# dream-faster/laplace-gnn-recommendation

Hardware: AMD Instinct MI355X
Metric: positive-edges/sec (train step) (higher is better)
Workload: dtype f32; 1 GPU; LightGCN train step, ONE synthetic bipartite graph 8000000x100000 users x items, 100000000 edges (seed 3, 64 user blocks), sharded by user over 1 GPU(s): 8000000 users / 100000000 edges per GPU, 3-layer D=128, global batch 131072 positive edges, on-device sampling, BPR + dense Adam; BASELINE.json configs[3]; parallelism=1 GPU

## Files before the change

### include/laplace_hip.h

```cpp
#ifndef LAPLACE_HIP_H
#define LAPLACE_HIP_H

#include <stddef.h>
#include <stdint.h>

#ifdef __cplusplus
extern "C" {
#endif

#define MI_ABI_VERSION 9

#define MI_ERR_BAD_ARG      (-1)
#define MI_ERR_TOO_LARGE    (-2)
#define MI_ERR_WORKSPACE    (-3)
#define MI_ERR_UNSUPPORTED  (-4)

typedef void* mi_stream_t;

int         mi_abi_version(void);
const char* mi_error_string(int code);

size_t mi_coo_to_csr_workspace_bytes(int64_t n_rows, int64_t nnz);
int    mi_coo_to_csr_i32(int64_t n_rows, int64_t n_cols, int64_t nnz,
                         const int64_t* row, const int64_t* col,
                         int32_t* rowptr, int32_t* col_out, int32_t* perm,
// ... 36 lines not shown

typedef struct mi_spmm_plan_info {
    int64_t n_long_rows, n_items, n_launch, nnz_long;
    int32_t chunk, band, n_bands, queue_len;
    int32_t queue_start[9];
    int32_t keys_in_second;
} mi_spmm_plan_info;

size_t mi_spmm_plan_workspace_bytes(int64_t n_rows, int64_t nnz);
int    mi_spmm_plan_count(int64_t n_rows, int64_t n_cols, const int32_t* rowptr, const int32_t* col,
                          int32_t chunk, int32_t band, void* ws, size_t ws_bytes,
                          mi_spmm_plan_info* info, mi_stream_t stream);
int    mi_spmm_plan_count_range(int64_t n_rows, int64_t n_cols, const int32_t* rowptr, const int32_t* col,
                                int32_t chunk, int32_t max_deg, int32_t band, void* ws, size_t ws_bytes,
                                mi_spmm_plan_info* info, mi_stream_t stream);
int    mi_spmm_plan_fill(int64_t n_rows, const int32_t* rowptr, const mi_spmm_plan_info* info,
                         mi_spmm_plan* plan, void* ws, size_t ws_bytes, mi_stream_t stream);
size_t mi_spmm_plan_pack_workspace_bytes(int64_t n_launch);
int    mi_spmm_plan_pack_entries(const mi_spmm_plan* plan, int64_t nnz_long, const int32_t* col, const float* val,
                                 int32_t values_only, void* ws, size_t ws_bytes, mi_stream_t stream);
size_t mi_spmm_workspace_bytes(const mi_spmm_plan* plan, int64_t d);

int mi_spmm_csr_f32(int64_t n_rows, int64_t d,
                    const int32_t* rowptr, const int32_t* col, const float* val,
                    const float* X, int64_t ldx,
                    float* Y, int64_t ldy,
                    const float* addend, int64_t lda,
                    float* S, int64_t lds, float scale,
                    const mi_spmm_plan* plan, void* ws, size_t ws_bytes,
                    mi_stream_t stream);
// ... 20 lines not shown
} mi_spmm_sweep;

typedef struct mi_spmm_ex {
    const int32_t* x_map;
    const int32_t* addend_map;
    const int32_t* row_list;
    const int32_t* n_list_dev;
    int64_t        n_list;
    const mi_adam_args* adam;
    int32_t        parts;
    int32_t        hot_rows;
    const mi_spmm_sweep* sweep;
    int32_t        hot_base;
    int32_t        hot_threads;
    const uint32_t* x_bits;
} mi_spmm_ex;
#define MI_SPMM_SHORT_ROWS 1
#define MI_SPMM_SPLIT_ROWS 2

int mi_spmm_csr_ex_f32(int64_t n_rows, int64_t d,
                       const int32_t* rowptr, const int32_t* col, const float* val,
                       const float* X, int64_t ldx,
                       float* Y, int64_t ldy,
                       const float* addend, int64_t lda,
                       float* S, int64_t lds, float scale,
                       const mi_spmm_plan* plan, const mi_spmm_ex* ex,
                       void* ws, size_t ws_bytes, mi_stream_t stream);

int mi_map_live_bits_i32(int64_t n, const int32_t* map, uint32_t* bits, mi_stream_t stream);

// ... 338 lines not shown
```

### laplace-gnn-recommendation_amd/_lib.py

```python
from __future__ import annotations

import ctypes
import os
from ctypes import POINTER, Structure, c_char_p, c_double, c_float, c_int32, c_int64, c_size_t, c_uint32, c_uint64, c_void_p

PKG_DIR = os.path.dirname(os.path.abspath(__file__))
LIB_PATH = os.environ.get("LAPLACE_HIP_LIB") or os.path.join(PKG_DIR, "liblaplace_hip.so")

MI_ABI_VERSION = 9
MI_SPMM_GROUP = 32


class MiError(RuntimeError):
    pass


class SpmmPlanStruct(Structure):
    _fields_ = [
        ("chunk", c_int32), ("n_long_rows", c_int32), ("n_items", c_int32), ("n_launch", c_int32),
        ("long_rows", c_void_p), ("item_ptr", c_void_p), ("items", c_void_p), ("long_index", c_void_p),
        ("band", c_int32), ("n_bands", c_int32),
        ("epos", c_void_p), ("ecol", c_void_p), ("eval", c_void_p),
    ]

# ... 6 lines not shown

class AdamArgs(Structure):
    _fields_ = [("p", c_void_p), ("ldp", c_int64), ("m", c_void_p), ("v", c_void_p), ("reg_w", c_void_p),
                ("lr", c_double), ("beta1", c_double), ("beta2", c_double), ("eps", c_double), ("step", c_int64)]


class SpmmSweepStruct(Structure):
    _fields_ = [("col", c_void_p), ("val", c_void_p), ("stream_ptr", c_void_p), ("slot_of", c_void_p),
                ("n_streams", c_int32), ("n_slots", c_int32), ("progress", c_void_p), ("epoch", c_int32), ("slack", c_int32)]


class SpmmExStruct(Structure):
    _fields_ = [("x_map", c_void_p), ("addend_map", c_void_p), ("row_list", c_void_p), ("n_list_dev", c_void_p),
                ("n_list", c_int64), ("adam", POINTER(AdamArgs)), ("parts", c_int32), ("hot_rows", c_int32),
                ("sweep", POINTER(SpmmSweepStruct)), ("hot_base", c_int32), ("hot_threads", c_int32),
                ("x_bits", c_void_p)]


MI_SPMM_SHORT_ROWS, MI_SPMM_SPLIT_ROWS = 1, 2
MI_ERR_UNSUPPORTED = -4
MI_ERR_WORKSPACE = -3
MI_TOPK_ITEMS_PREPARED = 1


class GemmProblem(Structure):
    _fields_ = [("trans_a", c_int32), ("trans_b", c_int32), ("m", c_int64), ("n", c_int64), ("k", c_int64),
                ("A", c_void_p), ("lda", c_int64), ("B", c_void_p), ("ldb", c_int64),
                ("k2", c_int64), ("A2", c_void_p), ("lda2", c_int64), ("B2", c_void_p), ("ldb2", c_int64),
                ("a_mask", c_void_p), ("bias", c_void_p), ("C", c_void_p), ("ldc", c_int64),
                ("accumulate", c_int32), ("act", c_int32)]

# ... 108 lines not shown

P = c_void_p
_PROTOTYPES = {
    "mi_abi_version": (c_int32, []),
    "mi_error_string": (c_char_p, [c_int32]),
    "mi_coo_to_csr_workspace_bytes": (c_size_t, [c_int64, c_int64]),
    "mi_coo_to_csr_i32": (c_int32, [c_int64, c_int64, c_int64, P, P, P, P, P, P, c_size_t, P]),
    "mi_csr_transpose_workspace_bytes": (c_size_t, [c_int64, c_int64]),
    "mi_csr_transpose_i32": (c_int32, [c_int64, c_int64, c_int64, P, P, P, P, P, P, c_size_t, P]),
    "mi_gather_f32": (c_int32, [c_int64, P, P, P, P]),
    "mi_gcn_norm_csr_f32": (c_int32, [c_int64, c_int64, P, P, P, P, P, P]),
    "mi_scale_csr_f32": (c_int32, [c_int64, c_int64, P, P, P, P, P, P, P]),
    "mi_spmm_plan_workspace_bytes": (c_size_t, [c_int64, c_int64]),
    "mi_spmm_plan_count": (c_int32, [c_int64, c_int64, P, P, c_int32, c_int32, P, c_size_t, POINTER(SpmmPlanInfo), P]),
    "mi_spmm_plan_count_range": (c_int32, [c_int64, c_int64, P, P, c_int32, c_int32, c_int32, P, c_size_t, POINTER(SpmmPlanInfo), P]),
    "mi_spmm_plan_fill": (c_int32, [c_int64, P, POINTER(SpmmPlanInfo), POINTER(SpmmPlanStruct), P, c_size_t, P]),
    "mi_spmm_workspace_bytes": (c_size_t, [POINTER(SpmmPlanStruct), c_int64]),
    "mi_spmm_plan_pack_workspace_bytes": (c_size_t, [c_int64]),
    "mi_spmm_plan_pack_entries": (c_int32, [POINTER(SpmmPlanStruct), c_int64, c_void_p, c_void_p, c_int32, c_void_p, c_size_t, c_void_p]),
    "mi_map_live_bits_i32": (c_int32, [c_int64, c_void_p, c_void_p, c_void_p]),
    "mi_spmm_csr_f32": (c_int32, [c_int64, c_int64, P, P, P, P, c_int64, P, c_int64, P, c_int64, P, c_int64,
                                  c_float, POINTER(SpmmPlanStruct), P, c_size_t, P]),
    "mi_spmm_csr_ex_f32": (c_int32, [c_int64, c_int64, P, P, P, P, c_int64, P, c_int64, P, c_int64, P, c_int64,
                                     c_float, POINTER(SpmmPlanStruct), POINTER(SpmmExStruct), P, c_size_t, P]),
    "mi_gather_rows_f32": (c_int32, [c_int64, P, P, c_int64, P, c_int64, P, c_int64, P, c_int64, c_int32, c_float, P]),
    "mi_scatter_rows_f32": (c_int32, [c_int64, P, P, c_int64, P, c_int64, P, c_int64, P, c_int64, P]),
    "mi_batch_nodes_workspace_bytes": (c_size_t, [c_int64]),
    "mi_batch_nodes_i32": (c_int32, [c_int64, c_int64, c_int64, P, P, P, P, P, P, P, c_size_t, P]),
    "mi_csr_expand_rows": (c_int32, [c_int64, P, P, c_int64, P]),
    "mi_sample_bpr_batch": (c_int32, [c_int64, c_int64, P, P, P, c_int64, c_int32, c_int32, c_uint64, c_uint64,
# ... 113 lines not shown
```

### laplace-gnn-recommendation_amd/csrc/spmm.hip

```cpp
#include "common.hpp"
#include "pairs.hpp"
#include <algorithm>
#include <rocprim/rocprim.hpp>

namespace {

#ifndef MI_SPMM_UNROLL
#define MI_SPMM_UNROLL 4
#endif
#ifndef MI_SPMM_UNROLL_ADAM
#define MI_SPMM_UNROLL_ADAM 8
#endif
#ifndef MI_SPMM_UNROLL_PAIR
#define MI_SPMM_UNROLL_PAIR 8
#endif
#ifndef MI_SPMM_ROWS_RPS
#define MI_SPMM_ROWS_RPS 1
#endif
#ifndef MI_SPMM_NT
#define MI_SPMM_NT 0
#endif
typedef float mi_f4v __attribute__((ext_vector_type(4)));
#ifndef MI_SPMM_SC1
#define MI_SPMM_SC1 6
// ... 36 lines not shown
    float4* v;
    const float* reg_w;
    MiAdamConsts adam;
};

struct Ex {
    const int32_t* x_map;
    const int32_t* addend_map;
    const int32_t* row_list;
    const int32_t* n_list_dev;
    const int32_t* long_index;
    int32_t parts;
    int32_t hot_base, hot_rows, hot_threads;
    const uint32_t* x_bits;
    uint8_t* slot_live;
};

template <int LPR>
__device__ __forceinline__ int wave_max_over_subgroups(int n) {
#pragma unroll
    for (int m = MI_WAVE / 2; m >= LPR; m >>= 1) n = max(n, __shfl_xor(n, m, MI_WAVE));
    return n;
}

template <int LPR, int VPL, int UNROLL, bool SPARSE>
__device__ __forceinline__ void subgroup_accumulate(const int32_t* __restrict__ col,
                                                    const float* __restrict__ val,
                                                    const float4* __restrict__ X4, int64_t ldx4, int d4,
                                                    int32_t beg, int n, int nmax, int li,
                                                    const int32_t* __restrict__ x_map, float4 (&acc)[VPL]) {
// ... 187 lines not shown
    const float4* X4; int64_t ldx4;
    Epilogue ep;
};
template <int LPR, int UNROLL>
__global__ __launch_bounds__(kBlock) void spmm_rows_pair_kernel(RowsSide a, RowsSide b, unsigned split) {
    const bool first = blockIdx.x < split;
#define MI_PICK(f) (first ? a.f : b.f)
    Epilogue ep;
    ep.Y = MI_PICK(ep.Y);           ep.ldy4 = MI_PICK(ep.ldy4);
    ep.addend = MI_PICK(ep.addend); ep.lda4 = MI_PICK(ep.lda4);
    ep.S = MI_PICK(ep.S);           ep.lds4 = MI_PICK(ep.lds4);
    ep.scale = MI_PICK(ep.scale);
    ep.streaming = MI_PICK(ep.streaming);
    ep.p = nullptr; ep.ldp4 = 0; ep.m = nullptr; ep.v = nullptr; ep.reg_w = nullptr;
    ep.adam = MiAdamConsts{};
    const Ex ex = {nullptr, nullptr, nullptr, nullptr, nullptr, 0, 0, 0, 0, nullptr, nullptr};
    spmm_rows_body<LPR, 1, UNROLL, MI_SPMM_ROWS_RPS, false, false>(first ? blockIdx.x : blockIdx.x - split, first ? split : gridDim.x - split,
                                                                  MI_PICK(n_out), MI_PICK(d4), MI_PICK(rowptr), MI_PICK(col), MI_PICK(val),
                                                                  MI_PICK(X4), MI_PICK(ldx4), ep, INT32_MAX, ex, 1);
#undef MI_PICK
}


struct HotRows {
    int32_t base, n;
    int32_t row_bytes;
};

#define MI_HOT_ENTRY(U)                                                                                              \
    "v_subrev_u32_e32 %[t2], %[hbase], %[c" #U "]\n"       \
    "v_cmp_gt_u32_e32 vcc, %[hn], %[t2]\n"                 \
// ... 572 lines not shown
    }
    __syncthreads();
    if (wave != 0 || lane >= LPR) return;
    float4 a[VPL];
    load_addend<LPR, VPL>(ep, ar, d4, lane, a);
#pragma unroll
    for (int v = 0; v < VPL; ++v) {
        float4 t = red[0][v][lane];
#pragma unroll
        for (int w = 1; w < kWavesPerBlock; ++w) t = mi_f4_add(t, red[w][v][lane]);
        acc[v] = t;
    }
    store_epilogue<LPR, VPL, ADAM>(ep, out_row, d4, lane, acc, a);
}

struct PlanWs {
    int32_t *is_long, *ldeg, *long_off, *lnz_off;
    int32_t* qstart;
    char* tmp; size_t tmp_bytes;
    int32_t *lrows, *lprefix;
    int32_t *flags, *seg_of;
    int32_t* seg_start;
    uint64_t *keys0, *keys1;
};

size_t plan_tmp_bytes(int64_t n_max) { return mi_align_up((size_t)n_max * 2 + ((size_t)32 << 20), 256); }

bool plan_carve(MiArena& ar, int64_t n_rows, int64_t nnz_total, int64_t n_long, int64_t nnz_long, int64_t n_seg,
                PlanWs& w) {
    const size_t n1 = (size_t)n_rows + 1;
// ... 6 lines not shown
    w.tmp = ar.take<char>(w.tmp_bytes);
    if (!w.is_long || !w.ldeg || !w.long_off || !w.lnz_off || !w.qstart || !w.tmp) return false;
    if (n_long < 0) return true;
    w.lrows = ar.take<int32_t>((size_t)n_long + 1);
    w.lprefix = ar.take<int32_t>((size_t)n_long + 1);
    w.flags = ar.take<int32_t>((size_t)(nnz_long > 0 ? nnz_long : 1));
    w.seg_of = ar.take<int32_t>((size_t)(nnz_long > 0 ? nnz_long : 1));
    if (!w.lrows || !w.lprefix || !w.flags || !w.seg_of) return false;
    if (n_seg < 0) return true;
    w.seg_start = ar.take<int32_t>((size_t)(n_seg > 0 ? n_seg : 1));
    w.keys0 = ar.take<uint64_t>((size_t)(n_seg > 0 ? n_seg : 1));
    w.keys1 = ar.take<uint64_t>((size_t)(n_seg > 0 ? n_seg : 1));
    return w.seg_start && w.keys0 && w.keys1;
}

__global__ void plan_flags_kernel(int64_t n_rows, const int32_t* __restrict__ rowptr, int32_t chunk, int32_t max_deg,
                                  int32_t* __restrict__ is_long, int32_t* __restrict__ ldeg) {
    int64_t r = (int64_t)blockIdx.x * blockDim.x + threadIdx.x;
    if (r > n_rows) return;
    const int32_t deg = (r < n_rows) ? rowptr[r + 1] - rowptr[r] : 0;
    const bool lg = deg > chunk && deg <= max_deg;
    is_long[r] = lg ? 1 : 0;
    ldeg[r] = lg ? deg : 0;
}

__global__ void plan_long_rows_kernel(int64_t n_rows, const int32_t* __restrict__ is_long,
                                      const int32_t* __restrict__ long_off, const int32_t* __restrict__ lnz_off,
                                      int32_t* __restrict__ lrows, int32_t* __restrict__ lprefix) {
    int64_t r = (int64_t)blockIdx.x * blockDim.x + threadIdx.x;
    if (r > n_rows) return;
    if (r == n_rows) {
        lprefix[long_off[r]] = lnz_off[r];
        return;
    }
    if (is_long[r]) {
        lrows[long_off[r]] = (int32_t)r;
// ... 144 lines not shown
}

dim3 plan_grid(int64_t n) { return dim3((unsigned)mi_ceil_div(n > 0 ? n : 1, 256)); }

#ifndef MI_SPMM_HOT_WAVES
#define MI_SPMM_HOT_WAVES 20
#endif
struct HotLaunch { int state = 0; int cus = 0; size_t lds_cap = 0; int occ_key = -1; int occ = 0; };

template <int LPR, int VPL, bool SPARSE, bool ADAM>
int launch_spmm_mode(int64_t n_rows, int d4, const int32_t* rowptr, const int32_t* col, const float* val,
                     const float4* X4, int64_t ldx4, const Epilogue& ep, const mi_spmm_plan* plan,
                     float4* partial, const Ex& ex, int64_t n_list, hipStream_t s, const mi_spmm_sweep* sweep) {
    constexpr int UNROLL = (VPL == 1) ? MI_SPMM_UNROLL : 4;
    constexpr int UNROLL_ROWS = (VPL == 1) ? (ADAM ? MI_SPMM_UNROLL_ADAM : MI_SPMM_UNROLL) : 4;
    constexpr int SG = (MI_WAVE / LPR) * kWavesPerBlock;
    constexpr int ROWS_RPS = MI_SPMM_ROWS_RPS;
#ifndef MI_SPMM_ITEMS_SLOTS
#define MI_SPMM_ITEMS_SLOTS 8
#endif
    constexpr int ITEMS_RPS = (SG >= MI_SPMM_ITEMS_SLOTS) ? 1 : MI_SPMM_ITEMS_SLOTS / SG;
    const int32_t chunk = plan ? plan->chunk : INT32_MAX;
    const bool listed = SPARSE && ex.row_list != nullptr;
    const bool do_short = (ex.parts & MI_SPMM_SHORT_ROWS) != 0, do_split = (ex.parts & MI_SPMM_SPLIT_ROWS) != 0;
    if (do_split && plan && plan->n_items > 0 && sweep) {
        if constexpr (VPL == 1 && LPR <= 32) {
            constexpr int NB = MI_WAVE / LPR;
            const int threads = 32 / NB * MI_WAVE;
            const size_t lds = (size_t)32 * 8 * LPR * sizeof(float4);
            auto kern = spmm_sweep_kernel<LPR, UNROLL, SPARSE>;
// ... 19 lines not shown
        bool done = false;
        xmap_form = false;
        if constexpr (SPARSE) {
            if (ex.x_map && ex.x_bits && ex.slot_live && plan->epos) {
                hipLaunchKernelGGL((spmm_items_xscan_kernel<LPR, VPL>),
                                   dim3((unsigned)mi_ceil_div(n_launch, (int64_t)(kWavesPerBlock * MI_WAVE))), dim3(kBlock), 0, s,
                                   n_launch, d4, reinterpret_cast<const int4*>(plan->items), plan->epos, plan->ecol, plan->eval,
                                   X4, ldx4, partial, ex.x_map, ex.x_bits, ex.slot_live, ep.streaming);
                done = xmap_form = true;
            }
        }
        if (!done)
            hipLaunchKernelGGL((spmm_items_kernel<LPR, VPL, UNROLL, ITEMS_RPS, SPARSE>), gi, dim3(kBlock), 0, s, n_launch,
                               plan->band > 0 ? 1 : 0, d4, reinterpret_cast<const int4*>(plan->items), plan->epos, ecol, eval,
                               X4, ldx4, partial, ex.x_map, ep.streaming);
    }
    const int64_t n_out = listed ? n_list : n_rows;
    bool short_done = false;
    if constexpr (!SPARSE && VPL == 1) {
        if (do_short && n_out > 0 && plan && ex.hot_rows != 0) {
            auto kern = spmm_rows_hot_kernel<LPR, UNROLL, ADAM>;
            static HotLaunch hl;
            const int thr_arg = ex.hot_threads & 0xFFF, waves_arg = ex.hot_threads >> 12;
            const int threads = thr_arg == 512 ? 512 : (thr_arg == 1024 ? 1024 : 256);
            const size_t row_bytes = (size_t)d4 * sizeof(float4);
            if (hl.state == 0) {
                hl.state = -1;
                hipDeviceProp_t prop;
                int dev = 0;
                if (hipGetDevice(&dev) == hipSuccess && hipGetDeviceProperties(&prop, dev) == hipSuccess) {
// ... 71 lines not shown
    if (n_rows < 0 || nnz < 0) return 0;
    const size_t n1 = (size_t)n_rows + 1, z = (size_t)(nnz > 0 ? nnz : 1);
    return 4 * mi_align_up(n1 * 4, 256) + 256 + plan_tmp_bytes(nnz > n_rows + 1 ? nnz : n_rows + 1) +
           2 * mi_align_up(n1 * 4, 256) + 3 * mi_align_up(z * 4, 256) + 2 * mi_align_up(z * 8, 256);
}

int mi_spmm_plan_count(int64_t n_rows, int64_t n_cols, const int32_t* rowptr, const int32_t* col,
                       int32_t chunk, int32_t band, void* ws, size_t ws_bytes, mi_spmm_plan_info* info,
                       mi_stream_t stream) {
    return mi_spmm_plan_count_range(n_rows, n_cols, rowptr, col, chunk, INT32_MAX, band, ws, ws_bytes, info, stream);
}

int mi_spmm_plan_count_range(int64_t n_rows, int64_t n_cols, const int32_t* rowptr, const int32_t* col,
                             int32_t chunk, int32_t max_deg, int32_t band, void* ws, size_t ws_bytes,
                             mi_spmm_plan_info* info, mi_stream_t stream) {
    MI_CHECK_ARG(n_rows >= 0 && n_cols >= 0 && rowptr && chunk > 0 && max_deg >= chunk && band >= 0 && ws && info);
    if (n_rows >= INT32_MAX || n_cols >= INT32_MAX) return MI_ERR_TOO_LARGE;
    hipStream_t s = (hipStream_t)stream;
    memset(info, 0, sizeof(*info));
    info->chunk = chunk;
    info->band = band;
    info->n_bands = band > 0 ? (int32_t)mi_ceil_div(n_cols > 0 ? n_cols : 1, band) : 0;
    int32_t nnz32 = 0;
    MI_HIP(hipMemcpyAsync(&nnz32, rowptr + n_rows, sizeof(int32_t), hipMemcpyDeviceToHost, s));
    MI_HIP(hipStreamSynchronize(s));
    const int64_t nnz = nnz32;
    MI_CHECK_ARG(band == 0 || col || nnz == 0);
    PlanWs w{};
    {
        MiArena ar(ws, ws_bytes);
        if (!plan_carve(ar, n_rows, nnz, -1, -1, -1, w)) return MI_ERR_WORKSPACE;
    }
    const int64_t n1 = n_rows + 1;
    hipLaunchKernelGGL(plan_flags_kernel, plan_grid(n1), dim3(256), 0, s, n_rows, rowptr, chunk, max_deg, w.is_long, w.ldeg);
    size_t tb = w.tmp_bytes;
    MI_HIP(rocprim::exclusive_scan(w.tmp, tb, w.is_long, w.long_off, 0, (size_t)n1, rocprim::plus<int32_t>(), s));
    tb = w.tmp_bytes;
    MI_HIP(rocprim::exclusive_scan(w.tmp, tb, w.ldeg, w.lnz_off, 0, (size_t)n1, rocprim::plus<int32_t>(), s));
    int32_t totals[2] = {0, 0};
    MI_HIP(hipMemcpyAsync(&totals[0], w.long_off + n_rows, sizeof(int32_t), hipMemcpyDeviceToHost, s));
    MI_HIP(hipMemcpyAsync(&totals[1], w.lnz_off + n_rows, sizeof(int32_t), hipMemcpyDeviceToHost, s));
    MI_HIP(hipStreamSynchronize(s));
    const int32_t n_long = totals[0], nnz_long = totals[1];
    info->n_long_rows = n_long;
    info->nnz_long = nnz_long;
    if (n_long == 0) return mi_launch_status();
    {
        MiArena ar(ws, ws_bytes);
        if (!plan_carve(ar, n_rows, nnz, n_long, nnz_long, -1, w)) return MI_ERR_WORKSPACE;
// ... 119 lines not shown
int mi_spmm_csr_ex_f32(int64_t n_rows, int64_t d, const int32_t* rowptr, const int32_t* col,
                       const float* val, const float* X, int64_t ldx, float* Y, int64_t ldy,
                       const float* addend, int64_t lda, float* S, int64_t lds, float scale,
                       const mi_spmm_plan* plan, const mi_spmm_ex* exh, void* ws, size_t ws_bytes,
                       mi_stream_t stream) {
    MI_CHECK_ARG(n_rows >= 0 && d > 0 && rowptr);
    if (n_rows == 0) return 0;
    if (d % 4 != 0 || d > 512) return MI_ERR_UNSUPPORTED;
    if (n_rows >= INT32_MAX) return MI_ERR_TOO_LARGE;
    const mi_adam_args* adam = exh ? exh->adam : nullptr;
    MI_CHECK_ARG(X && (Y || S || adam));
    MI_CHECK_ARG(ldx % 4 == 0 && ldx >= d && mi_aligned16(X));
    MI_CHECK_ARG(!Y || (ldy % 4 == 0 && ldy >= d && mi_aligned16(Y) && Y != X));
    MI_CHECK_ARG(!S || (lds % 4 == 0 && lds >= d && mi_aligned16(S) && S != X));
    MI_CHECK_ARG(!addend || (lda % 4 == 0 && lda >= d && mi_aligned16(addend)));
    Ex ex = {nullptr, nullptr, nullptr, nullptr, nullptr, MI_SPMM_SHORT_ROWS | MI_SPMM_SPLIT_ROWS, 0, 0, 0, nullptr, nullptr};
    int64_t n_list = 0;
    if (exh) {
        ex.x_map = exh->x_map;
        ex.addend_map = exh->addend_map;
        ex.row_list = exh->row_list;
        ex.n_list_dev = exh->n_list_dev;
        n_list = exh->n_list;
        if (exh->parts) {
            MI_CHECK_ARG((exh->parts & ~(MI_SPMM_SHORT_ROWS | MI_SPMM_SPLIT_ROWS)) == 0);
            ex.parts = exh->parts;
        }
        if (!ex.x_map && !ex.row_list && d <= 256) {
            MI_CHECK_ARG(exh->hot_base >= 0 && exh->hot_threads >= 0);
            ex.hot_base = exh->hot_base;
            ex.hot_rows = exh->hot_rows;
            ex.hot_threads = exh->hot_threads;
        }
        if (ex.row_list) {
            MI_CHECK_ARG(n_list >= 0 && !ex.addend_map);
            if (n_list == 0) return 0;
            if (plan && plan->n_long_rows > 0) {
                MI_CHECK_ARG(plan->long_index);
                ex.long_index = plan->long_index;
            }
        }
    }
    const mi_spmm_sweep* sweep = (exh && plan && plan->n_items > 0) ? exh->sweep : nullptr;
    if (sweep) {
        MI_CHECK_ARG(sweep->col && sweep->val && sweep->stream_ptr && sweep->slot_of);
        MI_CHECK_ARG(sweep->n_streams > 0 && sweep->n_streams % 32 == 0 && sweep->n_streams <= 32 * 32);
        MI_CHECK_ARG(sweep->n_slots > 0 && n_cols_ok(sweep) &&
                     (plan->items ? plan->n_items > 8 * sweep->n_slots : plan->n_items == 8 * sweep->n_slots));
        MI_CHECK_ARG(sweep->slack >= 0);
        if (d > 128) return MI_ERR_UNSUPPORTED;
    }
    float4* partial = nullptr;
// ... 100 lines not shown
```

### laplace-gnn-recommendation_amd/ops.py

```python
from __future__ import annotations

import ctypes
import os
from os import environ as _os_environ
from dataclasses import dataclass, field
from typing import Optional, Tuple

import torch as t
from torch import Tensor

from . import _lib
from ._lib import SpmmExStruct, SpmmPlanStruct, SpmmSweepStruct, check

DEFAULT_CHUNK = 256
DEFAULT_BAND = int(_os_environ.get("LAPLACE_SPMM_BAND", 16384))
MIN_BANDED_COLS = 131072

SPMM_EVENTS = None

SPMM_TWO_STREAMS = int(os.environ.get("LAPLACE_SPMM_TWO_STREAMS", "1") or 0)
PACK_ENTRIES = os.environ.get("LAPLACE_SPMM_PACK", "1") != "0"
X_RARE_BITS = os.environ.get("LAPLACE_X_RARE", "1") != "0"
_SIDE = {}


def _side_stream(device) -> "t.cuda.Stream":
    key = t.device(device).index
    if key not in _SIDE:
        _SIDE[key] = t.cuda.Stream(device=device)
    return _SIDE[key]

# ... 58 lines not shown

@dataclass
class SpmmPlan:
    struct: SpmmPlanStruct
    long_rows: Optional[Tensor]
    item_ptr: Optional[Tensor]
    items: Optional[Tensor]
    long_index: Optional[Tensor] = None
    partial: dict = field(default_factory=dict)
    sweep: Optional[SpmmSweepStruct] = None
    sweep_t: tuple = ()
    wide: Optional["SpmmPlan"] = None
    packed: tuple = ()
    packed_of: tuple = ()
    nnz_long: int = 0

    @property
    def n_long_rows(self) -> int:
        return int(self.struct.n_long_rows)

    @property
    def n_items(self) -> int:
        return int(self.struct.n_items)


@dataclass
class DeviceCSR:
    n_rows: int
    n_cols: int
    rowptr: Tensor
    col: Tensor
    val: Optional[Tensor] = None
    perm: Optional[Tensor] = None
    plan: Optional[SpmmPlan] = None
# ... 262 lines not shown
    st.n_items, st.n_launch = off + int(info.n_items), nlaunch
    st.long_rows, st.item_ptr, st.items, st.long_index = long_rows.data_ptr(), item_ptr.data_ptr(), items.data_ptr(), long_index.data_ptr()
    st.band, st.n_bands = int(info.band), int(info.n_bands)
    return SpmmPlan(st, long_rows, item_ptr, items, long_index, sweep=sw.sweep, sweep_t=sw.sweep_t)


HYBRID_TAIL_BAND = int(_os_environ.get("LAPLACE_HYBRID_TAIL_BAND", 16384))


import os as _os
SWEEP = _os.environ.get("LAPLACE_SWEEP", "1") != "0"
SWEEP_BAND = int(_os.environ.get("LAPLACE_SWEEP_BAND", SWEEP_BAND))
SWEEP_PACE = int(_os.environ.get("LAPLACE_SWEEP_PACE", SWEEP_PACE))


def build_spmm_plan(a: DeviceCSR, chunk: int = DEFAULT_CHUNK, band: Optional[int] = None, sweep: Optional[bool] = None) -> SpmmPlan:
    if (SWEEP if sweep is None else sweep) and band is None:
        plan = build_sweep_plan(a, chunk, band=SWEEP_BAND)
        if plan is not None:
            return plan
    L = _lib.lib()
    if band is None:
        band = DEFAULT_BAND if a.n_cols >= MIN_BANDED_COLS else 0
    dev = a.device
    ws = _ws(L.mi_spmm_plan_workspace_bytes(a.n_rows, a.nnz), dev)
    info = _lib.SpmmPlanInfo()
    check(L.mi_spmm_plan_count(a.n_rows, a.n_cols, _ptr(a.rowptr), _ptr(a.col), chunk, band, ws.data_ptr(), ws.numel(),
                               ctypes.byref(info), _stream()), "mi_spmm_plan_count")
    nl, nlaunch = int(info.n_long_rows), int(info.n_launch)
    long_rows = t.empty(max(nl, 1), dtype=t.int32, device=dev)
    item_ptr = t.empty(max(nl, 1) + 1, dtype=t.int32, device=dev)
    items = t.empty(4 * max(nlaunch, 1), dtype=t.int32, device=dev)
    long_index = t.empty(max(a.n_rows, 1), dtype=t.int32, device=dev)
    st = SpmmPlanStruct()
    st.long_rows, st.item_ptr, st.items = long_rows.data_ptr(), item_ptr.data_ptr(), items.data_ptr()
    st.long_index = long_index.data_ptr()
    check(L.mi_spmm_plan_fill(a.n_rows, _ptr(a.rowptr), ctypes.byref(info), ctypes.byref(st), ws.data_ptr(), ws.numel(),
                              _stream()), "mi_spmm_plan_fill")
    plan = SpmmPlan(st, long_rows, item_ptr, items, long_index)
    plan.nnz_long = int(info.nnz_long)
    del ws
    if PACK_ENTRIES and nlaunch > 0 and plan.nnz_long > 0 and a.val is not None:
        _pack_plan_entries(a, plan, values_only=False)
    return plan


def _pack_plan_entries(a: DeviceCSR, plan: SpmmPlan, values_only: bool) -> None:
    L = _lib.lib()
    dev, st = a.device, plan.struct
    if not values_only:
        plan.packed = (t.empty(int(st.n_launch), dtype=t.int32, device=dev), t.empty(plan.nnz_long, dtype=t.int32, device=dev),
                       t.empty(plan.nnz_long, dtype=t.float32, device=dev))
        st.epos, st.ecol, st.eval = (x.data_ptr() for x in plan.packed)
    ws = _ws(L.mi_spmm_plan_pack_workspace_bytes(int(st.n_launch)), dev)
    check(L.mi_spmm_plan_pack_entries(ctypes.byref(st), plan.nnz_long, _ptr(a.col), _ptr(a.val), 1 if values_only else 0,
                                      ws.data_ptr(), ws.numel(), _stream()), "mi_spmm_plan_pack_entries")
# ... 41 lines not shown
            raise ValueError(f"adam.p/m/v must be [{a.n_rows}, {d}]")
        rw = adam.get("reg_w")
        if rw is not None:
            _need(rw, t.float32, "adam.reg_w")
        adam_args = _lib.AdamArgs(p_.data_ptr(), ldp, m_.data_ptr(), v_.data_ptr(), _ptr(rw), float(adam["lr"]),
                                  float(adam.get("beta1", 0.9)), float(adam.get("beta2", 0.999)),
                                  float(adam.get("eps", 1e-8)), int(adam["step"]))
    ldy = _rows_ok(Y, "Y") if Y is not None else 0
    lda = _rows_ok(addend, "addend") if addend is not None else 0
    lds = _rows_ok(S, "S") if S is not None else 0
    if a.plan is None and (a.nnz >= PLAN_MIN_NNZ or row_list is not None):
        a.plan = build_spmm_plan(a)
    plan = a.plan
    if plan is not None and plan.sweep is not None and d > 128:
        if plan.wide is None:
            plan.wide = build_spmm_plan(a, chunk=int(plan.struct.chunk), sweep=False)
        plan = plan.wide
    L = _lib.lib()
    if plan is not None and plan.packed and plan.packed_of != (a.val.data_ptr(), a.val._version):
        _pack_plan_entries(a, plan, values_only=True)
    ws_ptr, ws_bytes = None, 0
    if plan is not None and plan.n_items > 0:
        if d not in plan.partial:
            plan.partial[d] = _ws(L.mi_spmm_workspace_bytes(ctypes.byref(plan.struct), d), a.device)
        ws_ptr, ws_bytes = plan.partial[d].data_ptr(), plan.partial[d].numel()
    col_ptr = _ptr(a.col) if a.nnz else a.rowptr.data_ptr()
    val_ptr = _ptr(a.val) if a.nnz else a.rowptr.data_ptr()
    ev = None
    if SPMM_EVENTS is not None:
        ev = (t.cuda.Event(enable_timing=True), t.cuda.Event(enable_timing=True))
        ev[0].record()
# ... 3 lines not shown
            and PERSISTENT_ROWS):
        hot_base, hot_rows = int(a.hot[0]), int(a.hot[1])
        if hot_rows == 0:
            hot_rows = -1
        if hot_base < 0 or hot_rows < -1 or hot_base + max(hot_rows, 0) > X.shape[0]:
            raise ValueError(f"hot rows [{hot_base}, {hot_base + hot_rows}) lie outside X ({X.shape[0]} rows)")

    x_bits = None
    if (x_rare and X_RARE_BITS and x_map is not None and row_list is None and sweep is None and plan is not None
            and plan.n_items > 0):
        x_bits = getattr(a, "_x_bits", None)
        if x_bits is None:
            x_bits = a._x_bits = t.empty((a.n_cols + 31) // 32, dtype=t.int32, device=a.device)
        check(L.mi_map_live_bits_i32(a.n_cols, _ptr(x_map), _ptr(x_bits), _stream()), "mi_map_live_bits_i32")

    def launch(parts: int, stream: int) -> None:
        exs = None
        if (x_map is not None or addend_map is not None or row_list is not None or adam_args is not None or parts
                or sweep is not None or hot_rows != 0 or HOT_THREADS):
            exs = SpmmExStruct(_ptr(x_map), _ptr(addend_map), _ptr(row_list), _ptr(n_list_dev),
                               row_list.numel() if row_list is not None else 0,
                               ctypes.pointer(adam_args) if adam_args is not None else None, parts, hot_rows,
                               ctypes.pointer(sweep) if sweep is not None else None, hot_base, HOT_THREADS, _ptr(x_bits))
        check(L.mi_spmm_csr_ex_f32(a.n_rows, d, _ptr(a.rowptr), col_ptr, val_ptr, X.data_ptr(), ldx,
                                   _ptr(Y), ldy, _ptr(addend), lda, _ptr(S), lds, float(scale),
                                   ctypes.byref(plan.struct) if plan is not None else None,
                                   ctypes.byref(exs) if exs is not None else None, ws_ptr, ws_bytes,
                                   stream), "mi_spmm_csr_ex_f32")

    if SPMM_TWO_STREAMS and plan is not None and plan.n_items > 0:
        cur = t.cuda.current_stream()
        side = _side_stream(a.device)
        side.wait_stream(cur)
        if SPMM_TWO_STREAMS == 2:
            launch(_lib.MI_SPMM_SPLIT_ROWS, cur.cuda_stream)
            launch(_lib.MI_SPMM_SHORT_ROWS, side.cuda_stream)
        else:
            launch(_lib.MI_SPMM_SHORT_ROWS, side.cuda_stream)
            launch(_lib.MI_SPMM_SPLIT_ROWS, cur.cuda_stream)
        cur.wait_stream(side)
    else:
        launch(0, _stream())
    if ev is not None:
        ev[1].record()
        kind = "sparse" if (x_map is not None or row_list is not None) else ("dense_adam" if adam is not None else "dense")
# ... 475 lines not shown
```

Measured before the change: 2.530 million positive-edges/s.

## Route medium-degree rows to a thin SpMM kernel splitting each row across waves

Adds a thin-row class to the SpMM plan: rows with degree between the chunk size and a threshold tied to the band count are taken out of the banded items path. They are handled by a new kernel that splits each row's nonzeros across one to four waves and reduces the partial sums in shared memory before the epilogue. The aim is to avoid the partial-buffer and item-scheduling overhead of the banded split path for moderately long rows. In exchange it adds a new launch, host-side nonzero and argsort work at plan build, and the ABI version is bumped.

```diff
diff --git a/include/laplace_hip.h b/include/laplace_hip.h
--- a/include/laplace_hip.h
+++ b/include/laplace_hip.h
@@ -8,7 +8,7 @@
 extern "C" {
 #endif
 
-#define MI_ABI_VERSION 9
+#define MI_ABI_VERSION 10
 
 #define MI_ERR_BAD_ARG      (-1)
 #define MI_ERR_TOO_LARGE    (-2)
@@ -75,6 +75,9 @@
 int    mi_spmm_plan_count_range(int64_t n_rows, int64_t n_cols, const int32_t* rowptr, const int32_t* col,
                                 int32_t chunk, int32_t max_deg, int32_t band, void* ws, size_t ws_bytes,
                                 mi_spmm_plan_info* info, mi_stream_t stream);
+int    mi_spmm_plan_count_thin(int64_t n_rows, int64_t n_cols, const int32_t* rowptr, const int32_t* col,
+                               int32_t chunk, int32_t thin_max, int32_t max_deg, int32_t band, void* ws, size_t ws_bytes,
+                               mi_spmm_plan_info* info, mi_stream_t stream);
 int    mi_spmm_plan_fill(int64_t n_rows, const int32_t* rowptr, const mi_spmm_plan_info* info,
                          mi_spmm_plan* plan, void* ws, size_t ws_bytes, mi_stream_t stream);
 size_t mi_spmm_plan_pack_workspace_bytes(int64_t n_launch);
@@ -125,6 +128,8 @@
     int32_t        hot_base;
     int32_t        hot_threads;
     const uint32_t* x_bits;
+    const int32_t* thin_rows;
+    int32_t        n_thin;
 } mi_spmm_ex;
 #define MI_SPMM_SHORT_ROWS 1
 #define MI_SPMM_SPLIT_ROWS 2
diff --git a/laplace-gnn-recommendation_amd/_lib.py b/laplace-gnn-recommendation_amd/_lib.py
--- a/laplace-gnn-recommendation_amd/_lib.py
+++ b/laplace-gnn-recommendation_amd/_lib.py
@@ -7,7 +7,7 @@
 PKG_DIR = os.path.dirname(os.path.abspath(__file__))
 LIB_PATH = os.environ.get("LAPLACE_HIP_LIB") or os.path.join(PKG_DIR, "liblaplace_hip.so")
 
-MI_ABI_VERSION = 9
+MI_ABI_VERSION = 10
 MI_SPMM_GROUP = 32
 
 
@@ -44,7 +44,7 @@
     _fields_ = [("x_map", c_void_p), ("addend_map", c_void_p), ("row_list", c_void_p), ("n_list_dev", c_void_p),
                 ("n_list", c_int64), ("adam", POINTER(AdamArgs)), ("parts", c_int32), ("hot_rows", c_int32),
                 ("sweep", POINTER(SpmmSweepStruct)), ("hot_base", c_int32), ("hot_threads", c_int32),
-                ("x_bits", c_void_p)]
+                ("x_bits", c_void_p), ("thin_rows", c_void_p), ("n_thin", c_int32)]
 
 
 MI_SPMM_SHORT_ROWS, MI_SPMM_SPLIT_ROWS = 1, 2
@@ -183,6 +183,7 @@
     "mi_spmm_plan_workspace_bytes": (c_size_t, [c_int64, c_int64]),
     "mi_spmm_plan_count": (c_int32, [c_int64, c_int64, P, P, c_int32, c_int32, P, c_size_t, POINTER(SpmmPlanInfo), P]),
     "mi_spmm_plan_count_range": (c_int32, [c_int64, c_int64, P, P, c_int32, c_int32, c_int32, P, c_size_t, POINTER(SpmmPlanInfo), P]),
+    "mi_spmm_plan_count_thin": (c_int32, [c_int64, c_int64, P, P, c_int32, c_int32, c_int32, c_int32, P, c_size_t, POINTER(SpmmPlanInfo), P]),
     "mi_spmm_plan_fill": (c_int32, [c_int64, P, POINTER(SpmmPlanInfo), POINTER(SpmmPlanStruct), P, c_size_t, P]),
     "mi_spmm_workspace_bytes": (c_size_t, [POINTER(SpmmPlanStruct), c_int64]),
     "mi_spmm_plan_pack_workspace_bytes": (c_size_t, [c_int64]),
diff --git a/laplace-gnn-recommendation_amd/csrc/spmm.hip b/laplace-gnn-recommendation_amd/csrc/spmm.hip
--- a/laplace-gnn-recommendation_amd/csrc/spmm.hip
+++ b/laplace-gnn-recommendation_amd/csrc/spmm.hip
@@ -74,6 +74,8 @@
     int32_t hot_base, hot_rows, hot_threads;
     const uint32_t* x_bits;
     uint8_t* slot_live;
+    const int32_t* thin_rows;
+    int32_t n_thin;
 };
 
 template <int LPR>
@@ -291,7 +293,7 @@
     ep.streaming = MI_PICK(ep.streaming);
     ep.p = nullptr; ep.ldp4 = 0; ep.m = nullptr; ep.v = nullptr; ep.reg_w = nullptr;
     ep.adam = MiAdamConsts{};
-    const Ex ex = {nullptr, nullptr, nullptr, nullptr, nullptr, 0, 0, 0, 0, nullptr, nullptr};
+    const Ex ex = {nullptr, nullptr, nullptr, nullptr, nullptr, 0, 0, 0, 0, nullptr, nullptr, nullptr, 0};
     spmm_rows_body<LPR, 1, UNROLL, MI_SPMM_ROWS_RPS, false, false>(first ? blockIdx.x : blockIdx.x - split, first ? split : gridDim.x - split,
                                                                   MI_PICK(n_out), MI_PICK(d4), MI_PICK(rowptr), MI_PICK(col), MI_PICK(val),
                                                                   MI_PICK(X4), MI_PICK(ldx4), ep, INT32_MAX, ex, 1);
@@ -894,6 +896,80 @@
     store_epilogue<LPR, VPL, ADAM>(ep, out_row, d4, lane, acc, a);
 }
 
+#ifndef MI_SPMM_UNROLL_THIN
+#define MI_SPMM_UNROLL_THIN 4
+#endif
+#ifndef MI_SPMM_THIN_WAVES
+#define MI_SPMM_THIN_WAVES 1
+#endif
+template <int LPR, int VPL, int UNROLL, bool SPARSE, bool ADAM>
+__global__ __launch_bounds__(kBlock) void spmm_thin_kernel(int64_t n_slots, int32_t waves, int d4,
+                                                           const int32_t* __restrict__ rowptr,
+                                                           const int32_t* __restrict__ col,
+                                                           const float* __restrict__ val,
+                                                           const float4* __restrict__ X4, int64_t ldx4,
+                                                           Epilogue ep, Ex ex) {
+    constexpr int NB = MI_WAVE / LPR, SG = NB * kWavesPerBlock;
+    __shared__ float4 red[SG][VPL][LPR];
+    const int lane = mi_lane();
+    const int li = lane % LPR;
+    const int wave = threadIdx.x / MI_WAVE;
+    const int sgi = wave * NB + lane / LPR;
+    const int pieces = waves * NB;
+    const int first_sg = (wave / waves) * pieces;
+    const int piece = sgi - first_sg;
+    const int64_t q = (int64_t)blockIdx.x * (kWavesPerBlock / waves) + wave / waves;
+    const bool listed = SPARSE && ex.row_list != nullptr;
+    int64_t r = 0, out_row = 0, ar = -1;
+    bool mine = q < n_slots;
+    if (mine) {
+        if (listed) {
+            if (ex.n_list_dev && q >= (int64_t)*ex.n_list_dev) mine = false;
+            if (mine) {
+                r = ex.row_list[q];
+                mine = ex.long_index[r] == -2;
+                out_row = ar = q;
+            }
+        } else {
+            r = ex.thin_rows[q];
+            out_row = r;
+            ar = ex.addend_map ? (int64_t)ex.addend_map[r] : r;
+        }
+    }
+    int32_t beg = 0;
+    int n = 0;
+    if (mine) {
+        const int32_t rb = rowptr[r];
+        const int32_t len = rowptr[r + 1] - rb;
+        const int32_t per = (len + pieces - 1) / pieces;
+        const int32_t b = min(piece * per, len);
+        beg = rb + b;
+        n = min(per, len - b);
+    }
+    const int nmax = wave_max_over_subgroups<LPR>(n);
+    float4 acc[VPL];
+    subgroup_accumulate<LPR, VPL, UNROLL, SPARSE>(col, val, X4, ldx4, d4, beg, n, nmax, li, ex.x_map, acc);
+#pragma unroll
+    for (int v = 0; v < VPL; ++v) red[sgi][v][li] = acc[v];
+    __syncthreads();
+    if (!mine || piece != 0) return;
+    float4 a[VPL];
+    load_addend<LPR, VPL>(ep, ar, d4, li, a);
+#pragma unroll
+    for (int v = 0; v < VPL; ++v) {
+        float4 t = red[first_sg][v][li];
+        for (int g = 1; g < pieces; ++g) t = mi_f4_add(t, red[first_sg + g][v][li]);
+        acc[v] = t;
+    }
+    store_epilogue<LPR, VPL, ADAM>(ep, out_row, d4, li, acc, a);
+}
+
+int32_t thin_waves() {
+    const char* e = getenv("LAPLACE_SPMM_THIN_WAVES");
+    const int v = e ? atoi(e) : MI_SPMM_THIN_WAVES;
+    return (v == 1 || v == 2) ? v : 4;
+}
+
 struct PlanWs {
     int32_t *is_long, *ldeg, *long_off, *lnz_off;
     int32_t* qstart;
@@ -930,12 +1006,12 @@
     return w.seg_start && w.keys0 && w.keys1;
 }
 
-__global__ void plan_flags_kernel(int64_t n_rows, const int32_t* __restrict__ rowptr, int32_t chunk, int32_t max_deg,
+__global__ void plan_flags_kernel(int64_t n_rows, const int32_t* __restrict__ rowptr, int32_t min_deg, int32_t max_deg,
                                   int32_t* __restrict__ is_long, int32_t* __restrict__ ldeg) {
     int64_t r = (int64_t)blockIdx.x * blockDim.x + threadIdx.x;
     if (r > n_rows) return;
     const int32_t deg = (r < n_rows) ? rowptr[r + 1] - rowptr[r] : 0;
-    const bool lg = deg > chunk && deg <= max_deg;
+    const bool lg = deg > min_deg && deg <= max_deg;
     is_long[r] = lg ? 1 : 0;
     ldeg[r] = lg ? deg : 0;
 }
@@ -1110,6 +1186,7 @@
                      float4* partial, const Ex& ex, int64_t n_list, hipStream_t s, const mi_spmm_sweep* sweep) {
     constexpr int UNROLL = (VPL == 1) ? MI_SPMM_UNROLL : 4;
     constexpr int UNROLL_ROWS = (VPL == 1) ? (ADAM ? MI_SPMM_UNROLL_ADAM : MI_SPMM_UNROLL) : 4;
+    constexpr int UNROLL_THIN = (VPL == 1) ? MI_SPMM_UNROLL_THIN : 4;
     constexpr int SG = (MI_WAVE / LPR) * kWavesPerBlock;
     constexpr int ROWS_RPS = MI_SPMM_ROWS_RPS;
 #ifndef MI_SPMM_ITEMS_SLOTS
@@ -1159,6 +1236,14 @@
             hipLaunchKernelGGL((spmm_items_kernel<LPR, VPL, UNROLL, ITEMS_RPS, SPARSE>), gi, dim3(kBlock), 0, s, n_launch,
                                plan->band > 0 ? 1 : 0, d4, reinterpret_cast<const int4*>(plan->items), plan->epos, ecol, eval,
                                X4, ldx4, partial, ex.x_map, ep.streaming);
+    }
+    if (do_split && ex.n_thin > 0) {
+        const int32_t waves = thin_waves();
+        const int64_t n_slots = listed ? n_list : (int64_t)ex.n_thin;
+        if (n_slots > 0)
+            hipLaunchKernelGGL((spmm_thin_kernel<LPR, VPL, UNROLL_THIN, SPARSE, ADAM>),
+                               dim3((unsigned)mi_ceil_div(n_slots, (int64_t)(kWavesPerBlock / waves))), dim3(kBlock), 0, s, n_slots,
+                               waves, d4, rowptr, col, val, X4, ldx4, ep, ex);
     }
     const int64_t n_out = listed ? n_list : n_rows;
     bool short_done = false;
@@ -1260,7 +1345,15 @@
 int mi_spmm_plan_count_range(int64_t n_rows, int64_t n_cols, const int32_t* rowptr, const int32_t* col,
                              int32_t chunk, int32_t max_deg, int32_t band, void* ws, size_t ws_bytes,
                              mi_spmm_plan_info* info, mi_stream_t stream) {
+    return mi_spmm_plan_count_thin(n_rows, n_cols, rowptr, col, chunk, 0, max_deg, band, ws, ws_bytes, info, stream);
+}
+
+int mi_spmm_plan_count_thin(int64_t n_rows, int64_t n_cols, const int32_t* rowptr, const int32_t* col,
+                            int32_t chunk, int32_t thin_max, int32_t max_deg, int32_t band, void* ws, size_t ws_bytes,
+                            mi_spmm_plan_info* info, mi_stream_t stream) {
     MI_CHECK_ARG(n_rows >= 0 && n_cols >= 0 && rowptr && chunk > 0 && max_deg >= chunk && band >= 0 && ws && info);
+    MI_CHECK_ARG(thin_max == 0 || (thin_max >= chunk && thin_max <= max_deg));
+    const int32_t min_deg = std::max(chunk, thin_max);
     if (n_rows >= INT32_MAX || n_cols >= INT32_MAX) return MI_ERR_TOO_LARGE;
     hipStream_t s = (hipStream_t)stream;
     memset(info, 0, sizeof(*info));
@@ -1278,7 +1371,7 @@
         if (!plan_carve(ar, n_rows, nnz, -1, -1, -1, w)) return MI_ERR_WORKSPACE;
     }
     const int64_t n1 = n_rows + 1;
-    hipLaunchKernelGGL(plan_flags_kernel, plan_grid(n1), dim3(256), 0, s, n_rows, rowptr, chunk, max_deg, w.is_long, w.ldeg);
+    hipLaunchKernelGGL(plan_flags_kernel, plan_grid(n1), dim3(256), 0, s, n_rows, rowptr, min_deg, max_deg, w.is_long, w.ldeg);
     size_t tb = w.tmp_bytes;
     MI_HIP(rocprim::exclusive_scan(w.tmp, tb, w.is_long, w.long_off, 0, (size_t)n1, rocprim::plus<int32_t>(), s));
     tb = w.tmp_bytes;
@@ -1428,7 +1521,7 @@
     MI_CHECK_ARG(!Y || (ldy % 4 == 0 && ldy >= d && mi_aligned16(Y) && Y != X));
     MI_CHECK_ARG(!S || (lds % 4 == 0 && lds >= d && mi_aligned16(S) && S != X));
     MI_CHECK_ARG(!addend || (lda % 4 == 0 && lda >= d && mi_aligned16(addend)));
-    Ex ex = {nullptr, nullptr, nullptr, nullptr, nullptr, MI_SPMM_SHORT_ROWS | MI_SPMM_SPLIT_ROWS, 0, 0, 0, nullptr, nullptr};
+    Ex ex = {nullptr, nullptr, nullptr, nullptr, nullptr, MI_SPMM_SHORT_ROWS | MI_SPMM_SPLIT_ROWS, 0, 0, 0, nullptr, nullptr, nullptr, 0};
     int64_t n_list = 0;
     if (exh) {
         ex.x_map = exh->x_map;
@@ -1446,10 +1539,15 @@
             ex.hot_rows = exh->hot_rows;
             ex.hot_threads = exh->hot_threads;
         }
+        if (exh->n_thin > 0) {
+            MI_CHECK_ARG(plan && exh->thin_rows);
+            ex.thin_rows = exh->thin_rows;
+            ex.n_thin = exh->n_thin;
+        }
         if (ex.row_list) {
             MI_CHECK_ARG(n_list >= 0 && !ex.addend_map);
             if (n_list == 0) return 0;
-            if (plan && plan->n_long_rows > 0) {
+            if (plan && (plan->n_long_rows > 0 || ex.n_thin > 0)) {
                 MI_CHECK_ARG(plan->long_index);
                 ex.long_index = plan->long_index;
             }
diff --git a/laplace-gnn-recommendation_amd/ops.py b/laplace-gnn-recommendation_amd/ops.py
--- a/laplace-gnn-recommendation_amd/ops.py
+++ b/laplace-gnn-recommendation_amd/ops.py
@@ -15,6 +15,7 @@
 DEFAULT_CHUNK = 256
 DEFAULT_BAND = int(_os_environ.get("LAPLACE_SPMM_BAND", 16384))
 MIN_BANDED_COLS = 131072
+THIN_PER_BAND = int(_os_environ.get("LAPLACE_SPMM_THIN", 2))
 
 SPMM_EVENTS = None
 
@@ -103,10 +104,20 @@
     packed: tuple = ()
     packed_of: tuple = ()
     nnz_long: int = 0
+    thin_rows: Optional[Tensor] = None
+    thin_max: int = 0
+
+    @property
+    def n_thin_rows(self) -> int:
+        return int(self.thin_rows.numel()) if self.thin_rows is not None else 0
+
+    @property
+    def n_split_rows(self) -> int:
+        return int(self.struct.n_long_rows)
 
     @property
     def n_long_rows(self) -> int:
-        return int(self.struct.n_long_rows)
+        return int(self.struct.n_long_rows) + self.n_thin_rows
 
     @property
     def n_items(self) -> int:
@@ -399,7 +410,8 @@
 SWEEP_PACE = int(_os.environ.get("LAPLACE_SWEEP_PACE", SWEEP_PACE))
 
 
-def build_spmm_plan(a: DeviceCSR, chunk: int = DEFAULT_CHUNK, band: Optional[int] = None, sweep: Optional[bool] = None) -> SpmmPlan:
+def build_spmm_plan(a: DeviceCSR, chunk: int = DEFAULT_CHUNK, band: Optional[int] = None, sweep: Optional[bool] = None,
+                    thin_max: Optional[int] = None) -> SpmmPlan:
     if (SWEEP if sweep is None else sweep) and band is None:
         plan = build_sweep_plan(a, chunk, band=SWEEP_BAND)
         if plan is not None:
@@ -407,11 +419,16 @@
     L = _lib.lib()
     if band is None:
         band = DEFAULT_BAND if a.n_cols >= MIN_BANDED_COLS else 0
+        if thin_max is None and band > 0:
+            thin_max = THIN_PER_BAND * ((a.n_cols + band - 1) // band)
+    thin_max = int(thin_max or 0)
+    if thin_max <= chunk:
+        thin_max = 0
     dev = a.device
     ws = _ws(L.mi_spmm_plan_workspace_bytes(a.n_rows, a.nnz), dev)
     info = _lib.SpmmPlanInfo()
-    check(L.mi_spmm_plan_count(a.n_rows, a.n_cols, _ptr(a.rowptr), _ptr(a.col), chunk, band, ws.data_ptr(), ws.numel(),
-                               ctypes.byref(info), _stream()), "mi_spmm_plan_count")
+    check(L.mi_spmm_plan_count_thin(a.n_rows, a.n_cols, _ptr(a.rowptr), _ptr(a.col), chunk, thin_max, 2 ** 31 - 1, band,
+                                    ws.data_ptr(), ws.numel(), ctypes.byref(info), _stream()), "mi_spmm_plan_count_thin")
     nl, nlaunch = int(info.n_long_rows), int(info.n_launch)
     long_rows = t.empty(max(nl, 1), dtype=t.int32, device=dev)
     item_ptr = t.empty(max(nl, 1) + 1, dtype=t.int32, device=dev)
@@ -425,6 +442,14 @@
     plan = SpmmPlan(st, long_rows, item_ptr, items, long_index)
     plan.nnz_long = int(info.nnz_long)
     del ws
+    plan.thin_max = thin_max
+    if thin_max > 0 and a.n_rows > 0:
+        deg = a.rowptr[1:] - a.rowptr[:-1]
+        rows = t.nonzero((deg > chunk) & (deg <= thin_max)).view(-1)
+        if rows.numel() > 0:
+            rows = rows[t.argsort(deg[rows], descending=True, stable=True)]
+            long_index[rows] = -2
+            plan.thin_rows = rows.to(t.int32).contiguous()
     if PACK_ENTRIES and nlaunch > 0 and plan.nnz_long > 0 and a.val is not None:
         _pack_plan_entries(a, plan, values_only=False)
     return plan
@@ -496,7 +521,7 @@
     plan = a.plan
     if plan is not None and plan.sweep is not None and d > 128:
         if plan.wide is None:
-            plan.wide = build_spmm_plan(a, chunk=int(plan.struct.chunk), sweep=False)
+            plan.wide = build_spmm_plan(a, chunk=int(plan.struct.chunk), sweep=False, thin_max=0)
         plan = plan.wide
     L = _lib.lib()
     if plan is not None and plan.packed and plan.packed_of != (a.val.data_ptr(), a.val._version):
@@ -530,21 +555,24 @@
             x_bits = a._x_bits = t.empty((a.n_cols + 31) // 32, dtype=t.int32, device=a.device)
         check(L.mi_map_live_bits_i32(a.n_cols, _ptr(x_map), _ptr(x_bits), _stream()), "mi_map_live_bits_i32")
 
+    n_thin = plan.n_thin_rows if plan is not None else 0
+
     def launch(parts: int, stream: int) -> None:
         exs = None
         if (x_map is not None or addend_map is not None or row_list is not None or adam_args is not None or parts
-                or sweep is not None or hot_rows != 0 or HOT_THREADS):
+                or sweep is not None or hot_rows != 0 or HOT_THREADS or n_thin):
             exs = SpmmExStruct(_ptr(x_map), _ptr(addend_map), _ptr(row_list), _ptr(n_list_dev),
                                row_list.numel() if row_list is not None else 0,
                                ctypes.pointer(adam_args) if adam_args is not None else None, parts, hot_rows,
-                               ctypes.pointer(sweep) if sweep is not None else None, hot_base, HOT_THREADS, _ptr(x_bits))
+                               ctypes.pointer(sweep) if sweep is not None else None, hot_base, HOT_THREADS, _ptr(x_bits),
+                               _ptr(plan.thin_rows) if n_thin else None, n_thin)
         check(L.mi_spmm_csr_ex_f32(a.n_rows, d, _ptr(a.rowptr), col_ptr, val_ptr, X.data_ptr(), ldx,
                                    _ptr(Y), ldy, _ptr(addend), lda, _ptr(S), lds, float(scale),
                                    ctypes.byref(plan.struct) if plan is not None else None,
                                    ctypes.byref(exs) if exs is not None else None, ws_ptr, ws_bytes,
                                    stream), "mi_spmm_csr_ex_f32")
 
-    if SPMM_TWO_STREAMS and plan is not None and plan.n_items > 0:
+    if SPMM_TWO_STREAMS and plan is not None and (plan.n_items > 0 or n_thin > 0):
         cur = t.cuda.current_stream()
         side = _side_stream(a.device)
         side.wait_stream(cur)
```

Measured after the change: 2.753 million positive-edges/s (median of 6 runs). 8.8% higher.
